# Jutho/KrylovKit.jl

Measured on NVIDIA H100. Metric: eigsolve_lanczos_operator_applications_per_sec, higher is better.
Workload: dtype f64

## Files before the change

krylovkit.jl_b200/csrc/basis.cu:

```cuda
#include "tsk.cuh"
#include <cmath>
#include <algorithm>

int32_t b2k_enqueue_dot(b2k_ctx* ctx, const void* q, void* x, int64_t n, const void* qprev,
                        int sprev_slot, int slot, int accum_slot);
int32_t b2k_enqueue_axpy_dev(b2k_ctx* ctx, void* x, const void* q, int s_slot, int64_t n);
int32_t b2k_enqueue_apply(b2k_ctx* ctx, const b2k_op* op, const VecRef& x, const VecRef& y,
                          double a0, double a1, bool shifted, const VecRef* dotv, int dot_slot);

using namespace tsk;

namespace {


template <typename T, bool UPDATE, bool PROJECT>
__global__ void __launch_bounds__(NTHREADS, 1)
k_phase(const __grid_constant__ PhaseParams<T> p, const __grid_constant__ ColList cl) {
    extern __shared__ __align__(128) uint8_t smem[];
    SmemView sm(smem);
    const int64_t ntiles = (p.n + Cfg<T>::R - 1) / Cfg<T>::R;
    const bool ragged = (p.n % Cfg<T>::R) != 0 && ((ntiles - 1) % gridDim.x) == blockIdx.x;
    pipe_setup(sm, ragged);
    Pipe st;
    if (threadIdx.x >= NCONS) producer_phase<T>(p, cl, sm, st);
    else consumer_phase<T, UPDATE, PROJECT>(p, sm, st);
}

template <typename T>
struct FusedParams {
    PhaseParams<T> ph[3];
    int32_t kind[3];
    int32_t nph;
    unsigned* barrier;
    unsigned barrier_base;
    const int* stop;
    FinalizeParams fin;
    PeerStep ps;
    unsigned long long* trace;
};

template <typename T>
__device__ __forceinline__ void peer_boundary(const FusedParams<T>& fp, int i, uint8_t* smem) {
    __threadfence();
    asm volatile("fence.proxy.async;" ::: "memory");
    __syncthreads();
    int* flag = reinterpret_cast<int*>(smem + OFF_RED + 256);
    if (threadIdx.x == 0) {
        const unsigned old = atomicAdd(fp.barrier, 1u);
        *flag = (old == fp.barrier_base + (unsigned)(i + 1) * gridDim.x - 1u);
    }
    __syncthreads();
    const PeerDev& pd = fp.ps.pd;
    const int tid = threadIdx.x;
    if (fp.ph[i].part_h == nullptr) {
        const unsigned long long sq = fp.ps.seq_norm;
        if (*flag && tid < 32) {
            __threadfence();
            double a = (tid < 16) ? partial_lane_sum(fp.ph[i].part_n, gridDim.x, 1, tid, 16) : 0.0;
            for (int o = 8; o > 0; o >>= 1) a += __shfl_xor_sync(0xffffffffu, a, o);
            if (tid == 0) peer_publish1(pd, PEER_CH_NORM, sq, a);
        }
        peer_wait(pd, PEER_CH_NORM, sq, tid);
        __syncthreads();
        return;
    }
    const unsigned long long seq = fp.ps.seq_coef[i];
    if (*flag && tid < NCONS) {
        __threadfence();
        const int k = fp.ph[i].k;
        const int L = coef_lanes(k);
        const int j = tid / L, l = tid % L;
        const bool valid = j < k;
        const double a = coef_colsum(fp.ph[i].part_h, gridDim.x, B2K_KSTRIDE, j, l, L, valid);
        if (valid && l == 0)
            for (int p = 0; p < pd.nranks; ++p) peer_slot(pd, p, PEER_CH_COEF, seq, pd.rank)[j] = a;
        __threadfence_system();
        named_bar_sync(1, NCONS);
        if (tid < pd.nranks) st_release_sys_u64(peer_flag(pd, tid, PEER_CH_COEF, seq, pd.rank), seq);
    }
    peer_wait(pd, PEER_CH_COEF, seq, tid);
    __syncthreads();
}

template <typename T>
__global__ void __launch_bounds__(NTHREADS, 1)
k_gs_fused(const __grid_constant__ FusedParams<T> fp, const __grid_constant__ ColList cl) {
    extern __shared__ __align__(128) uint8_t smem[];
    if (fp.stop && *reinterpret_cast<const volatile int*>(fp.stop)) {
        if (threadIdx.x == 0 && fp.nph > 1) atomicAdd(fp.barrier, (unsigned)(fp.nph - 1));
        return;
    }
    SmemView sm(smem);
    const bool tr0 = fp.trace && blockIdx.x == 0 && threadIdx.x == 0;
    if (tr0) b2k_trace(fp.trace, 10);
    const int64_t n = fp.ph[0].n;
    const int64_t ntiles = (n + Cfg<T>::R - 1) / Cfg<T>::R;
    const bool ragged = (n % Cfg<T>::R) != 0 && ((ntiles - 1) % gridDim.x) == blockIdx.x;
    pipe_setup(sm, ragged);
    Pipe st;
    const bool prod = threadIdx.x >= NCONS;
    if (fp.ps.on && fp.ps.seq_alpha && !prod) {
        peer_wait(fp.ps.pd, PEER_CH_ALPHA, fp.ps.seq_alpha, threadIdx.x);
        named_bar_sync(1, NCONS);
    }
    if (tr0) b2k_trace(fp.trace, 11);
    for (int i = 0; i < fp.nph; ++i) {
        if (prod) {
            producer_phase<T>(fp.ph[i], cl, sm, st);
        } else {
            if (fp.kind[i] == 0) consumer_phase<T, false, true>(fp.ph[i], sm, st);
            else if (fp.kind[i] == 1) consumer_phase<T, true, true>(fp.ph[i], sm, st);
            else consumer_phase<T, true, false>(fp.ph[i], sm, st);
        }
        if (tr0) b2k_trace(fp.trace, 12 + i);
        if (i + 1 < fp.nph) {
            if (fp.ps.on) peer_boundary<T>(fp, i, smem);
            else grid_barrier(fp.barrier, fp.barrier_base + (unsigned)(i + 1) * gridDim.x);
            if (tr0) b2k_trace(fp.trace, 15 + i);
        }
    }
    if (fp.fin.enabled && !prod) {
        double* sh = reinterpret_cast<double*>(smem + OFF_RED);
        int* flag = reinterpret_cast<int*>(smem + OFF_RED + 256);
        if (fp.ps.on) __threadfence_system();
        else __threadfence();
        named_bar_sync(1, NCONS);
        if (threadIdx.x == 0) {
            const unsigned t = atomicInc(fp.fin.ticket, gridDim.x - 1);
            *flag = (t == gridDim.x - 1);
        }
        named_bar_sync(1, NCONS);
        if (*flag) {
            __threadfence();
            if (fp.trace && threadIdx.x == 0) b2k_trace(fp.trace, 18);
            finalize_block(fp.fin, threadIdx.x, sh, fp.ps.on ? &fp.ps : nullptr);
            if (fp.trace && threadIdx.x == 0) b2k_trace(fp.trace, 19);
        }
    }
}

__global__ void __launch_bounds__(NCONS)
k_finalize(const double* __restrict__ A, const double* __restrict__ B, const double* __restrict__ N, int G,
           int stride, int k, double* __restrict__ res, int off, int noff) {
    __shared__ double sh[2];
    FinalizeParams f;
    f.A = A; f.B = B; f.N = N; f.G = G; f.stride = stride; f.k = k; f.res = res; f.off = off; f.noff = noff;
    f.rec = nullptr; f.alpha_col = -1; f.tol = 0.0; f.stop = nullptr; f.ticket = nullptr; f.enabled = 1;
    f.peer = 0; f.G_local = G; f.norm_done = 0;
    finalize_block(f, threadIdx.x, sh);
}

__global__ void k_lanczos_seed(double* rec, double beta, int* stop) {
    rec[2] = beta;
    rec[3] = 1.0 / beta;
    rec[4] = beta * beta;
    *stop = 0;
}

template <typename T>
__global__ void k_res_to_vec(const double* __restrict__ res, T* __restrict__ out, int k,
                             T alpha) {
    const int j = blockIdx.x * blockDim.x + threadIdx.x;
    if (j < k) out[j] = alpha * (T)res[j];
}

struct TransformParams {
    void* base;
    int64_t ld, n;
    int32_t m, keep, ldu;
    const double* U;
    int32_t u_in_smem;
};

constexpr int TR_OFF_U = NS * SLOT_BYTES;
constexpr int TR_U_BYTES = 232448 - TR_OFF_U - 256;
constexpr int TR_OFF_BAR = TR_OFF_U + TR_U_BYTES;
constexpr int TR_SMEM = TR_OFF_BAR + 2 * NS * 8;
constexpr int TJ = 36;
constexpr int TR_THREADS = NCONS + 32;

template <typename T, bool USM>
__global__ void __launch_bounds__(TR_THREADS, 1)
k_transform(const __grid_constant__ TransformParams p, const __grid_constant__ ColList cl) {
    using CF = Cfg<T>;
    using V16 = typename CF::V16;
    constexpr int R = CF::R, C = CF::C, VEC = CF::VEC;
    extern __shared__ __align__(128) uint8_t smem[];
    const uint32_t ring = smem_u32(smem);
    const uint32_t full = smem_u32(smem + TR_OFF_BAR), empty = full + NS * 8;
    T* Us = reinterpret_cast<T*>(smem + TR_OFF_U);
    const int pitch = ((p.keep + VEC - 1) / VEC) * VEC;
    if (threadIdx.x == 0) {
        for (int i = 0; i < NS; ++i) {
            mbar_init(full + 8 * i, 1);
            mbar_init(empty + 8 * i, NCONS / 32);
        }
        fence_mbar_init();
    }
// ... 779 lines not shown
    if (kind == 0) return launch_phase_t<T, false, true>(ctx, p, cl, grid);
    if (kind == 1) return launch_phase_t<T, true, true>(ctx, p, cl, grid);
    return launch_phase_t<T, true, false>(ctx, p, cl, grid);
}

template <typename T>
int grid_for_rows(const b2k_ctx* ctx, int64_t n) {
    int64_t ntiles = (n + Cfg<T>::R - 1) / Cfg<T>::R;
    if (ntiles < 1) ntiles = 1;
    return (int)std::min<int64_t>(ntiles, ctx->num_sms);
}

bool g_coop_launch = true;

template <typename T>
int32_t launch_fused(b2k_ctx* ctx, FusedParams<T>& fp, const ColList& cl, int grid) {
    fp.barrier = ctx->d_sync + 1;
    fp.barrier_base = ctx->barrier_base;
    ctx->barrier_base += (unsigned)(fp.nph - 1) * (unsigned)grid;
    void* args[] = {(void*)&fp, (void*)&cl};
    if (g_coop_launch)
        B2K_CUDA(ctx, cudaLaunchCooperativeKernel((const void*)k_gs_fused<T>, dim3(grid), dim3(NTHREADS),
                                                  args, SMEM_BYTES, ctx->stream));
    else
        k_gs_fused<T><<<grid, NTHREADS, SMEM_BYTES, ctx->stream>>>(fp, cl);
    B2K_LAUNCH_CHECK(ctx);
    return B2K_OK;
}

int32_t enqueue_finalize(b2k_ctx* ctx, const double* A, const double* B, const double* N, int G,
                         int k, int off, int noff) {
    if (k > NCONS) return b2k_fail(ctx, B2K_ENOTSUP, "finalize: more than %d coefficients per pass", NCONS);
    k_finalize<<<1, NCONS, 0, ctx->stream>>>(A, B, N, G, B2K_KSTRIDE, k, ctx->d_res, off, noff);
    B2K_LAUNCH_CHECK(ctx);
    return B2K_OK;
}

bool g_l2_hints = true;
int g_chain_mode = 0;

struct Panel {
    void* base;
    int64_t ld, n;
    int32_t sharded;
    std::vector<int32_t> idx;
};

int32_t make_panel(b2k_ctx* ctx, const b2k_vec* cols, int32_t k, Panel* pn) {
    int32_t sp = 0;
    B2K_TRY(b2k_resolve_cols(ctx, cols, k, &sp, &pn->idx));
    if (k == 0) {
        pn->base = nullptr;
        return B2K_OK;
    }
    const B2kSpace& s = ctx->spaces[sp];
    pn->base = s.base;
    pn->ld = s.ld;
    pn->n = s.n;
    pn->sharded = s.sharded;
    return B2K_OK;
}

template <typename T>
void fill_cols(ColList& cl, const std::vector<int32_t>& idx, int off, int cnt) {
    for (int i = 0; i < cnt; ++i) cl.c[i] = idx[off + i];
}

template <typename T>
PhaseParams<T> base_params(const Panel& pn, int k, const void* x, void* xout) {
    PhaseParams<T> p;
    memset(&p, 0, sizeof(p));
    p.base = (const T*)pn.base;
    p.ld = pn.ld;
    p.n = pn.n;
    p.k = k;
    p.x = (const T*)x;
    p.xout = (T*)xout;
    p.nvec = 1;
    p.beta_mode = 1;
    p.betax = (T)1;
    p.alphac = (T)1;
    p.l2_hints = g_l2_hints ? 1 : 0;
    return p;
}

template <typename T>
int32_t project_t(b2k_ctx* ctx, const Panel& pn, const VecRef& x, int k, int res_off) {
    const int grid = grid_for_rows<T>(ctx, pn.n);
    const int KC = kcap<T>();
    for (int off = 0; off < k; off += KC) {
        const int kk = std::min(KC, k - off);
        ColList cl;
        fill_cols<T>(cl, pn.idx, off, kk);
        PhaseParams<T> p = base_params<T>(pn, kk, x.ptr, nullptr);
        p.part_h = b2k_part_set(ctx, 0);
        const int pr = b2k_prof_begin(ctx, 3, (kk + 1.0) * sizeof(T) * (double)pn.n);
        B2K_TRY((launch_phase_t<T, false, true>(ctx, p, cl, grid)));
        b2k_prof_end(ctx, pr);
        B2K_TRY(enqueue_finalize(ctx, b2k_part_set(ctx, 0), nullptr, nullptr, grid, kk,
                                 res_off + off, 0));
    }
    return B2K_OK;
}

template <typename T>
int32_t unproject_t(b2k_ctx* ctx, const Panel& pn, const VecRef& y, int k, const double* dcoef,
                    const T* coef_t, double alpha, double beta, double* part_n) {
    const int grid = grid_for_rows<T>(ctx, pn.n);
    const int KC = kcap<T>();
    int off = 0;
    do {
        const int kk = std::min(KC, k - off);
        ColList cl;
        fill_cols<T>(cl, pn.idx, off, kk);
        PhaseParams<T> p = base_params<T>(pn, kk, y.ptr, y.ptr);
        p.store_x = 1;
        p.coef = dcoef ? dcoef + off : nullptr;
        p.coef_t = coef_t ? coef_t + off : nullptr;
        p.coef_sets = 1;
        p.coef_stride = 0;
        p.alphac = (T)alpha;
        if (off == 0) {
            p.beta_mode = beta == 0.0 ? 0 : (beta == 1.0 ? 1 : 2);
            p.betax = (T)beta;
        }
        p.part_n = (off + kk >= k) ? part_n : nullptr;
        const int pr = b2k_prof_begin(ctx, 4, (kk + 2.0) * sizeof(T) * (double)pn.n);
        B2K_TRY((launch_phase_t<T, true, false>(ctx, p, cl, grid)));
        b2k_prof_end(ctx, pr);
        off += kk;
    } while (off < k);
    return B2K_OK;
}

template <typename T>
int32_t cgs_fused_t(b2k_ctx* ctx, const Panel& pn, const VecRef& v, int k, int passes,
                    bool use_coop) {
    const int grid = grid_for_rows<T>(ctx, pn.n);
    ColList cl;
    fill_cols<T>(cl, pn.idx, 0, k);
    double* PA = b2k_part_set(ctx, 0);
    double* PB = b2k_part_set(ctx, 1);
    double* PN = b2k_part_set(ctx, 2);
    FusedParams<T> fp;
    memset(&fp, 0, sizeof(fp));
    int nph = 0;
    {
        PhaseParams<T> p = base_params<T>(pn, k, v.ptr, nullptr);
        p.part_h = PA;
        fp.ph[nph] = p; fp.kind[nph] = 0; ++nph;
    }
    if (passes == 2) {
        PhaseParams<T> p = base_params<T>(pn, k, v.ptr, v.ptr);
        p.store_x = 1;
        p.coef = PA; p.coef_sets = grid; p.coef_stride = B2K_KSTRIDE;
        p.alphac = (T)-1;
        p.part_h = PB;
        fp.ph[nph] = p; fp.kind[nph] = 1; ++nph;
    }
    {
        PhaseParams<T> p = base_params<T>(pn, k, v.ptr, v.ptr);
        p.store_x = 1;
        p.coef = (passes == 2) ? PB : PA; p.coef_sets = grid; p.coef_stride = B2K_KSTRIDE;
        p.alphac = (T)-1;
        p.part_n = PN;
        fp.ph[nph] = p; fp.kind[nph] = 2; ++nph;
// ... 292 lines not shown
    for (int j = 0; j < k; ++j) h_host[j] = ctx->h_res[j];
    nrm = sqrt(ctx->h_res[k]);
    if (nrm_out) *nrm_out = nrm;
    if (passes_out) *passes_out = passes;
    return B2K_OK;
}

extern "C" int32_t b2k_lanczos_expand(b2k_ctx* ctx, const b2k_op* op, const b2k_vec* cols,
                                      int32_t k, b2k_vec r, b2k_vec w, double beta_old,
                                      int32_t alg, double eta, double* alpha_out,
                                      double* beta_out) {
    if (!ctx || !op || !cols || k < 1 || !alpha_out || !beta_out) return B2K_EINVAL;
    if (alg < B2K_CGS || alg > B2K_MGS2B)
        return b2k_fail(ctx, B2K_EINVAL, "lanczos_expand: unknown orthogonalizer %d", alg);
    if (cols[k] != r) return b2k_fail(ctx, B2K_EINVAL, "lanczos_expand: cols[k] must be r");
    if (beta_old == 0.0) return b2k_fail(ctx, B2K_EINVAL, "lanczos_expand: beta_old == 0");
    Panel pn;
    B2K_TRY(make_panel(ctx, cols, k + 1, &pn));
    VecRef rv, rw, vprev;
    B2K_TRY(b2k_resolve(ctx, r, &rv));
    B2K_TRY(b2k_resolve(ctx, w, &rw));
    B2K_TRY(b2k_resolve(ctx, cols[k - 1], &vprev));
    if (rv.n != pn.n || rw.n != pn.n) return b2k_fail(ctx, B2K_EDIM, "lanczos_expand: length mismatch");
    for (int j = 0; j <= k; ++j)
        if (cols[j] == w) return b2k_fail(ctx, B2K_EINVAL, "lanczos_expand: w aliases the basis");
    const bool f64 = ctx->dtype == B2K_F64;
    const int K1 = k + 1;
    const double eps = f64 ? 2.220446049250313e-16 : 1.1920929e-07;
    const int S_H = 0;
    const int S_N = K1;
    const int S_A0 = K1 + 1;

    B2K_TRY(b2k_vec_scale(ctx, r, r, 1.0 / beta_old));

    if (alg == B2K_CGS || alg == B2K_CGS2 || alg == B2K_CGSIR) {
        B2K_TRY(b2k_enqueue_apply(ctx, op, rv, rw, 0.0, 1.0, false, &rv, S_A0));
        B2K_TRY(b2k_allreduce(ctx, ctx->d_res + S_A0, 1, pn.sharded));
        const bool one_pass = K1 <= (f64 ? kcap<double>() : kcap<float>());
        const bool defer_alpha = (alg == B2K_CGS2) && one_pass;
        double alpha = 0.0;
        if (!defer_alpha) {
            B2K_TRY(b2k_fetch_results(ctx, S_A0 + 1, 0));
            alpha = ctx->h_res[S_A0];
        }
        if (alg == B2K_CGS) {
            B2K_TRY(b2k_vec_axpy2(ctx, w, cols[k - 1], -beta_old, r, -alpha));
            B2K_TRY(b2k_enqueue_dot(ctx, nullptr, rw.ptr, pn.n, nullptr, -1, S_N, -1));
            B2K_TRY(b2k_allreduce(ctx, ctx->d_res + S_N, 1, pn.sharded));
            B2K_TRY(b2k_fetch_results(ctx, S_N + 1, 0));
            *alpha_out = alpha;
            *beta_out = sqrt(ctx->h_res[S_N]);
            return B2K_OK;
        }
        double ab2 = alpha * alpha + beta_old * beta_old;
        double beta = 0.0, nold = 0.0;
        bool first = true;
        for (;;) {
            const bool fusable = fused_ok(ctx, K1, pn.sharded, ctx->dtype);
            const bool prologue = first;
            if (alg == B2K_CGSIR && first) {
                B2K_TRY(b2k_vec_axpy2(ctx, w, cols[k - 1], -beta_old, r, -alpha));
                B2K_TRY(b2k_enqueue_dot(ctx, nullptr, rw.ptr, pn.n, nullptr, -1, S_N, -1));
                B2K_TRY(b2k_allreduce(ctx, ctx->d_res + S_N, 1, pn.sharded));
                B2K_TRY(b2k_fetch_results(ctx, S_N + 1, 0));
                beta = sqrt(ctx->h_res[S_N]);
                nold = sqrt(beta * beta + ab2);
                first = false;
                if (!(eps < beta && beta < eta * nold)) break;
                nold = beta;
                continue;
            }
            if (fusable) {
                const int grid = f64 ? grid_for_rows<double>(ctx, pn.n) : grid_for_rows<float>(ctx, pn.n);
                ColList cl;
                for (int i = 0; i < K1; ++i) cl.c[i] = pn.idx[i];
                double* PA = b2k_part_set(ctx, 0);
                double* PN = b2k_part_set(ctx, 2);
#define BUILD_AND_LAUNCH(T)                                                                   \
    {                                                                                         \
        FusedParams<T> fp;                                                                    \
        memset(&fp, 0, sizeof(fp));                                                           \
        PhaseParams<T> a = base_params<T>(pn, K1, rw.ptr, rw.ptr);                            \
        if (prologue) {                                                                       \
            a.nvec = 3; a.e1 = (const T*)vprev.ptr; a.e2 = (const T*)rv.ptr;                  \
            a.c1 = (T)(-beta_old); a.c2 = (T)(-alpha); a.store_x = 1;                         \
            if (defer_alpha) a.c2_dev = ctx->d_res + S_A0;                                    \
        }                                                                                     \
        a.part_h = PA;                                                                        \
        PhaseParams<T> c = base_params<T>(pn, K1, rw.ptr, rw.ptr);                            \
        c.store_x = 1; c.coef = PA; c.coef_sets = grid; c.coef_stride = B2K_KSTRIDE;          \
        c.alphac = (T)-1; c.part_n = PN;                                                      \
        fp.ph[0] = a; fp.kind[0] = 0; fp.ph[1] = c; fp.kind[1] = 2; fp.nph = 2;               \
        const int pr = b2k_prof_begin(ctx, 1, (2.0 * K1 + 3.0) * sizeof(T) * (double)pn.n);   \
        if (g_use_coop) { B2K_TRY(launch_fused<T>(ctx, fp, cl, grid)); }                      \
        else {                                                                                \
            B2K_TRY(launch_phase<T>(ctx, fp.ph[0], cl, 0, grid));                             \
            B2K_TRY(launch_phase<T>(ctx, fp.ph[1], cl, 2, grid));                             \
        }                                                                                     \
        b2k_prof_end(ctx, pr);                                                                \
    }
                if (f64) BUILD_AND_LAUNCH(double) else BUILD_AND_LAUNCH(float)
#undef BUILD_AND_LAUNCH
                B2K_TRY(enqueue_finalize(ctx, PA, nullptr, PN, grid, K1, S_H, S_N));
                B2K_TRY(b2k_fetch_results(ctx, S_A0 + 1, 0));
                if (defer_alpha) alpha = ctx->h_res[S_A0];
            } else if (one_pass) {
                const int grid = f64 ? grid_for_rows<double>(ctx, pn.n) : grid_for_rows<float>(ctx, pn.n);
                ColList cl;
                for (int i = 0; i < K1; ++i) cl.c[i] = pn.idx[i];
                double* PA = b2k_part_set(ctx, 0);
                double* PN = b2k_part_set(ctx, 2);
#define SPLIT_SWEEPS(T)                                                                       \
    {                                                                                         \
        PhaseParams<T> a = base_params<T>(pn, K1, rw.ptr, rw.ptr);                            \
        if (prologue) {                                                                       \
            a.nvec = 3; a.e1 = (const T*)vprev.ptr; a.e2 = (const T*)rv.ptr;                  \
            a.c1 = (T)(-beta_old); a.c2 = (T)(-alpha); a.store_x = 1;                         \
            if (defer_alpha) a.c2_dev = ctx->d_res + S_A0;                                    \
        }                                                                                     \
        a.part_h = PA;                                                                        \
        const int pr = b2k_prof_begin(ctx, 1, (2.0 * K1 + 3.0) * sizeof(T) * (double)pn.n);   \
        B2K_TRY(launch_phase<T>(ctx, a, cl, 0, grid));                                        \
        B2K_TRY(enqueue_finalize(ctx, PA, nullptr, nullptr, grid, K1, S_H, S_N));             \
        B2K_TRY(b2k_allreduce(ctx, ctx->d_res + S_H, K1, pn.sharded));                        \
        PhaseParams<T> c = base_params<T>(pn, K1, rw.ptr, rw.ptr);                            \
        c.store_x = 1; c.coef = ctx->d_res + S_H; c.coef_sets = 1; c.coef_stride = 0;         \
        c.alphac = (T)-1; c.part_n = PN;                                                      \
        B2K_TRY(launch_phase<T>(ctx, c, cl, 2, grid));                                        \
        b2k_prof_end(ctx, pr);                                                                \
    }
                if (f64) SPLIT_SWEEPS(double) else SPLIT_SWEEPS(float)
#undef SPLIT_SWEEPS
                k_finalize<<<1, NCONS, 0, ctx->stream>>>(PN, nullptr, PN, grid, B2K_KSTRIDE, 0, ctx->d_res, 0, S_N);
                B2K_LAUNCH_CHECK(ctx);
                B2K_TRY(b2k_allreduce(ctx, ctx->d_res + S_N, 1, pn.sharded));
                B2K_TRY(b2k_fetch_results(ctx, S_A0 + 1, 0));
                if (defer_alpha) alpha = ctx->h_res[S_A0];
            } else {
                if (prologue) B2K_TRY(b2k_vec_axpy2(ctx, w, cols[k - 1], -beta_old, r, -alpha));
                if (f64) B2K_TRY(cgs_pass_unfused_t<double>(ctx, pn, rw, K1, S_H, S_N));
                else B2K_TRY(cgs_pass_unfused_t<float>(ctx, pn, rw, K1, S_H, S_N));
                B2K_TRY(b2k_fetch_results(ctx, S_N + 1, 0));
            }
            alpha += ctx->h_res[S_H + k];
            beta = sqrt(ctx->h_res[S_N]);
            first = false;
            if (alg == B2K_CGS2) break;
            if (!(eps < beta && beta < eta * nold)) break;
            nold = beta;
        }
        *alpha_out = alpha;
        *beta_out = beta;
        return B2K_OK;
    }

    B2K_TRY(b2k_enqueue_apply(ctx, op, rv, rw, 0.0, 1.0, false, nullptr, -1));
    B2K_TRY(b2k_vec_axpby(ctx, w, cols[k - 1], -beta_old, 1.0));
    B2K_TRY(b2k_enqueue_dot(ctx, rv.ptr, rw.ptr, pn.n, nullptr, -1, S_A0, -1));
    B2K_TRY(b2k_allreduce(ctx, ctx->d_res + S_A0, 1, pn.sharded));
    B2K_TRY(b2k_enqueue_axpy_dev(ctx, rw.ptr, rv.ptr, S_A0, pn.n));
    double alpha = 0.0, beta = 0.0;
    if (alg == B2K_MGS) {
        B2K_TRY(b2k_enqueue_dot(ctx, nullptr, rw.ptr, pn.n, nullptr, -1, S_N, -1));
        B2K_TRY(b2k_allreduce(ctx, ctx->d_res + S_N, 1, pn.sharded));
        B2K_TRY(b2k_fetch_results(ctx, S_A0 + 1, 0));
        alpha = ctx->h_res[S_A0];
        beta = sqrt(ctx->h_res[S_N]);
    } else if (alg == B2K_MGS2B) {
        if (fused_ok(ctx, K1, pn.sharded, ctx->dtype)) {
            if (f64) B2K_TRY(cgs_fused_t<double>(ctx, pn, rw, K1, 1, g_use_coop));
            else B2K_TRY(cgs_fused_t<float>(ctx, pn, rw, K1, 1, g_use_coop));
        } else {
            if (f64) B2K_TRY(cgs_pass_unfused_t<double>(ctx, pn, rw, K1, S_H, S_N));
            else B2K_TRY(cgs_pass_unfused_t<float>(ctx, pn, rw, K1, S_H, S_N));
        }
        B2K_TRY(b2k_fetch_results(ctx, S_A0 + 1, 0));
        alpha = ctx->h_res[S_A0] + ctx->h_res[S_H + k];
        beta = sqrt(ctx->h_res[S_N]);
    } else if (alg == B2K_MGS2) {
        B2K_TRY(mgs_sweep(ctx, pn, rw, K1, S_H, -1));
        B2K_TRY(b2k_enqueue_dot(ctx, nullptr, rw.ptr, pn.n, nullptr, -1, S_N, -1));
        B2K_TRY(b2k_allreduce(ctx, ctx->d_res + S_N, 1, pn.sharded));
        B2K_TRY(b2k_fetch_results(ctx, S_A0 + 1, 0));
        alpha = ctx->h_res[S_A0] + ctx->h_res[S_H + k];
        beta = sqrt(ctx->h_res[S_N]);
    } else {
        B2K_TRY(b2k_enqueue_dot(ctx, nullptr, rw.ptr, pn.n, nullptr, -1, S_N, -1));
        B2K_TRY(b2k_allreduce(ctx, ctx->d_res + S_N, 1, pn.sharded));
        B2K_TRY(b2k_fetch_results(ctx, S_A0 + 1, 0));
        alpha = ctx->h_res[S_A0];
        beta = sqrt(ctx->h_res[S_N]);
        double nold = sqrt(beta * beta + alpha * alpha + beta_old * beta_old);
        while (eps < beta && beta < eta * nold) {
            nold = beta;
            B2K_TRY(mgs_sweep(ctx, pn, rw, K1, S_H, -1));
            B2K_TRY(b2k_enqueue_dot(ctx, nullptr, rw.ptr, pn.n, nullptr, -1, S_N, -1));
            B2K_TRY(b2k_allreduce(ctx, ctx->d_res + S_N, 1, pn.sharded));
            B2K_TRY(b2k_fetch_results(ctx, S_N + 1, 0));
            alpha += ctx->h_res[S_H + k];
            beta = sqrt(ctx->h_res[S_N]);
        }
    }
    *alpha_out = alpha;
    *beta_out = beta;
    return B2K_OK;
}

bool g_use_chain = true;

bool chain_ok(const b2k_ctx* ctx, const b2k_op* op, const b2k_vec* cols, int32_t k, int32_t nsteps, int32_t alg,
              double beta_old) {
    if (!g_use_chain || !g_use_coop || (alg != B2K_CGS2 && alg != B2K_MGS2B) || nsteps < 1 || nsteps > B2K_MAX_CHAIN)
        return false;
    int64_t op_rows = 0, op_cols = 0;
    int32_t op_kind = -1;
    if (b2k_op_info(op, &op_rows, &op_cols, nullptr, &op_kind) != B2K_OK) return false;
    if ((op_kind != 0 && op_kind != 2) || beta_old == 0.0 || !(beta_old == beta_old)) return false;
    const int32_t sp = B2K_VEC_SPACE(cols[k]);
    if (sp < 0 || sp >= (int32_t)ctx->spaces.size()) return false;
    const B2kSpace& s = ctx->spaces[sp];
    if (ctx->nranks > 1) {
        if (!s.sharded || !b2k_peer_ok(ctx) || !b2k_op_has_peer_halo(op) || op_rows != s.n) return false;
    } else if (op_rows != s.n || op_cols != s.n) {
        return false;
    }
    const int C = ctx->dtype == B2K_F64 ? 8 : 16;
    const int K1 = k + nsteps;
    return (K1 + C - 1) / C <= NS && K1 <= MAXCH * C && K1 <= PEER_SLOT;
}

template <typename T>
int32_t chain_step_gs(b2k_ctx* ctx, const Panel& pn, int K1, const VecRef& rw, const VecRef& vprev,
                      const VecRef& rv, double* rec_prev, double* rec, double tol, const PeerStep* psp,
                      bool scale_after) {
    const int grid = grid_for_rows<T>(ctx, pn.n);
    ColList cl;
    for (int i = 0; i < K1; ++i) cl.c[i] = pn.idx[i];
    double* PA = b2k_part_set(ctx, 0);
    double* PN = b2k_part_set(ctx, 2);
    FusedParams<T> fp;
    memset(&fp, 0, sizeof(fp));
    PhaseParams<T> a = base_params<T>(pn, K1, rw.ptr, rw.ptr);
    a.nvec = 3; a.e1 = (const T*)vprev.ptr; a.e2 = (const T*)rv.ptr; a.store_x = 1;
    a.c1_dev = rec_prev + 2;
    a.c2_dev = rec + 0;
    a.part_h = PA;
    PhaseParams<T> c = base_params<T>(pn, K1, rw.ptr, rw.ptr);
    c.store_x = 1; c.coef = PA; c.coef_sets = grid; c.coef_stride = B2K_KSTRIDE;
    c.alphac = (T)-1; c.part_n = PN;
    fp.ph[0] = a; fp.kind[0] = 0; fp.ph[1] = c; fp.kind[1] = 2; fp.nph = 2;
    if (scale_after) {
        PhaseParams<T> sc = base_params<T>(pn, 0, rw.ptr, rw.ptr);
        sc.store_x = 1; sc.beta_mode = 2; sc.scale_mode = 1;
        sc.scale_norm = PN; sc.scale_G = grid; sc.scale_stride = 1; sc.scale_tol = tol;
        fp.ph[2] = sc; fp.kind[2] = 2; fp.nph = 3;
    }
    fp.stop = reinterpret_cast<const int*>(ctx->d_sync + B2K_SYNC_STOP);
    fp.trace = ctx->d_trace;
    fp.fin.A = PA; fp.fin.B = nullptr; fp.fin.N = PN; fp.fin.G = grid; fp.fin.stride = B2K_KSTRIDE;
    fp.fin.k = K1; fp.fin.res = nullptr; fp.fin.off = 0; fp.fin.noff = 0; fp.fin.rec = rec;
    fp.fin.alpha_col = K1 - 1; fp.fin.tol = tol;
    fp.fin.stop = reinterpret_cast<int*>(ctx->d_sync + B2K_SYNC_STOP);
    fp.fin.ticket = ctx->d_sync + B2K_SYNC_GSFIN; fp.fin.enabled = 1;
    fp.fin.peer = 0; fp.fin.G_local = grid; fp.fin.norm_done = 0;
    if (psp && psp->on) {
        const PeerStep& ps = *psp;
        fp.ps = ps;
        char* win = b2k_peer_local(ctx);
        auto slot = [&](int ch, unsigned long long seq) {
            return reinterpret_cast<double*>(win + PEER_OFF_SLOTS) + (size_t)((ch * 2 + (int)(seq & 1ull)) * PEER_MAXR) * PEER_SLOT;
        };
        fp.ph[0].c2_dev = slot(PEER_CH_ALPHA, ps.seq_alpha);
        fp.ph[0].c2_sets = ps.pd.nranks;
        fp.ph[0].c2_stride = PEER_SLOT;
        fp.ph[1].coef = slot(PEER_CH_COEF, ps.seq_coef[0]);
        fp.ph[1].coef_sets = ps.pd.nranks;
        fp.ph[1].coef_stride = PEER_SLOT;
        fp.fin.A = fp.ph[1].coef; fp.fin.G = ps.pd.nranks; fp.fin.stride = PEER_SLOT; fp.fin.peer = 1;
        const int last = fp.nph - 1;
        if (scale_after) {
            fp.ph[2].scale_norm = slot(PEER_CH_NORM, ps.seq_norm);
            fp.ph[2].scale_G = ps.pd.nranks;
            fp.ph[2].scale_stride = PEER_SLOT;
            fp.fin.norm_done = 1;
        }
        if (ps.seq_halo) {
            fp.ph[last].send_lo = ps.send_lo;
            fp.ph[last].send_hi = ps.send_hi;
            fp.ph[last].halo_dn = ps.send_lo ? reinterpret_cast<T*>(ps.pd.win[ps.pd.rank - 1] + ps.dn_off) : nullptr;
            fp.ph[last].halo_up = ps.send_hi ? reinterpret_cast<T*>(ps.pd.win[ps.pd.rank + 1] + ps.up_off) : nullptr;
        }
    }
    const int pr = b2k_prof_begin(ctx, 1, (2.0 * K1 + 3.0) * sizeof(T) * (double)pn.n);
    B2K_TRY(launch_fused<T>(ctx, fp, cl, grid));
    b2k_prof_end(ctx, pr);
    return B2K_OK;
}

int32_t lanczos_chain(b2k_ctx* ctx, const b2k_op* op, b2k_vec* cols, int32_t k, int32_t nsteps,
                      double beta_old, double tol, int32_t alg, double* alphas_out, double* betas_out,
                      int32_t* steps_done, b2k_vec* r_out) {
    const bool f64 = ctx->dtype == B2K_F64;
    const int32_t space = B2K_VEC_SPACE(cols[k]);
    double* rec0 = ctx->d_steps;
    int* d_stop = reinterpret_cast<int*>(ctx->d_sync + B2K_SYNC_STOP);
    {
        VecRef t;
        for (int i = 0; i <= k; ++i) B2K_TRY(b2k_resolve(ctx, cols[i], &t));
    }
    k_lanczos_seed<<<1, 1, 0, ctx->stream>>>(rec0, beta_old, d_stop);
    B2K_LAUNCH_CHECK(ctx);
    const bool inplace = g_chain_mode == 1;
    std::vector<b2k_vec> touched, Vh, Wh;
    touched.push_back(cols[k]);
    int32_t enq = 0, rc = B2K_OK;
    const bool dist = ctx->nranks > 1;
    unsigned long long halo_seq = 0;
    if (inplace) B2K_TRY(b2k_vec_scale(ctx, cols[k], cols[k], 1.0 / beta_old));
    for (int32_t i = 0; i < nsteps; ++i) {
        const int32_t K = k + i;
        const b2k_vec R = cols[K];
        b2k_vec V = R, W = -1;
        if (!inplace) {
            rc = b2k_vec_alloc(ctx, space, &V);
            if (rc != B2K_OK) break;
            touched.push_back(V);
        }
        rc = b2k_vec_alloc(ctx, space, &W);
        if (rc != B2K_OK) break;
        touched.push_back(W);
        VecRef rR, rV, rW, vprev;
        rc = b2k_resolve(ctx, R, &rR);
        if (rc == B2K_OK) rc = b2k_resolve(ctx, V, &rV);
        if (rc == B2K_OK) rc = b2k_resolve(ctx, W, &rW);
        if (rc == B2K_OK) rc = b2k_resolve(ctx, cols[K - 1], &vprev);
        if (rc != B2K_OK) break;
        double* rec_prev = rec0 + (size_t)B2K_REC * i;
        double* rec = rec0 + (size_t)B2K_REC * (i + 1);
        const bool scale_after = inplace && (i + 1 < nsteps);
        SpmvFuse fz;
        memset(&fz, 0, sizeof(fz));
        if (!inplace) {
            fz.xscale = rec_prev + 3;
            fz.vout = rV.ptr;
        }
        fz.stop = d_stop;
        fz.dot_self = 1;
        fz.l2_hints = g_l2_hints ? 1 : 0;
        fz.trace = ctx->d_trace;
        if (alg == B2K_MGS2B) {
            fz.dot_sub_vec = vprev.ptr;
            fz.dot_sub_scale = rec_prev + 2;
        }
        PeerStep ps;
        memset(&ps, 0, sizeof(ps));
        if (dist) {
            ps.on = 1;
// ... 294 lines not shown
```

krylovkit.jl_b200/csrc/tsk.cuh:

```cuda
#pragma once
#include "common.cuh"

namespace tsk {

template <typename T> struct Cfg;
template <> struct Cfg<double> {
    static constexpr int R = 256, C = 8, VEC = 2;
    using V16 = double2;
    __device__ static __forceinline__ void unpack(const double2& v, double* o) { o[0] = v.x; o[1] = v.y; }
};
template <> struct Cfg<float> {
    static constexpr int R = 256, C = 16, VEC = 4;
    using V16 = float4;
    __device__ static __forceinline__ void unpack(const float4& v, float* o) {
        o[0] = v.x; o[1] = v.y; o[2] = v.z; o[3] = v.w;
    }
};

constexpr int NS = 12;
constexpr int NW = 3;
constexpr int NCONS = 256;
constexpr int NPROD = 4;
constexpr int NTHREADS = NCONS + 32 * NPROD;
constexpr int MAXCH = 16;
constexpr int SLOT_BYTES = 16384;
static_assert(NS % NPROD == 0, "a ring slot must always be refilled by the same producer warp");

template <typename T> constexpr int kcap() { return MAXCH * Cfg<T>::C; }

constexpr int OFF_RING = 0;
constexpr int OFF_WRING = NS * SLOT_BYTES;
constexpr int WSLOT_MAX = 3 * 256 * 8;
constexpr int OFF_W1 = OFF_WRING + NW * WSLOT_MAX;
constexpr int OFF_CS = OFF_W1 + 2 * 256 * 8;
constexpr int OFF_RED = OFF_CS + 1024;
constexpr int OFF_BAR = OFF_RED + 512;
constexpr int SMEM_BYTES = OFF_BAR + (2 * NS + 2 * NW) * 8;

struct ColList {
    int32_t c[256];
};

template <typename T>
struct PhaseParams {
    const T* base;
    int64_t ld;
    int64_t n;
    int32_t k;
    const T* x;
    T* xout;
    const T* e1;
    const T* e2;
    T c1, c2;
    const double* c1_dev;
    const double* c2_dev;
    int32_t c2_sets;
    int32_t c2_stride;
    T* halo_dn;
    T* halo_up;
    int64_t send_lo, send_hi;
    int32_t scale_mode;
    const double* scale_norm;
    int32_t scale_G, scale_stride;
    double scale_tol;
    int32_t nvec;
    int32_t store_x;
    int32_t l2_hints;
    const double* coef;
    const T* coef_t;
    int32_t coef_sets;
    int32_t coef_stride;
    T alphac, betax;
    int32_t beta_mode;
    double* part_h;
    double* part_n;
};

struct Pipe {
    uint32_t s = 0, ph = 0, ws = 0, wph = 0;
    uint32_t g = 0;
};

struct SmemView {
    uint8_t* raw;
    uint32_t ring, wring, full, empty, wfull, wempty;
    __device__ explicit SmemView(uint8_t* p) : raw(p) {
        ring = smem_u32(p + OFF_RING);
        wring = smem_u32(p + OFF_WRING);
        full = smem_u32(p + OFF_BAR);
        empty = full + NS * 8;
        wfull = empty + NS * 8;
        wempty = wfull + NW * 8;
    }
};

__device__ __forceinline__ void pipe_setup(const SmemView& sm, bool zero_ring) {
    if (threadIdx.x == 0) {
        for (int i = 0; i < NS; ++i) {
            mbar_init(sm.full + 8 * i, 1);
            mbar_init(sm.empty + 8 * i, NCONS / 32);
        }
        for (int i = 0; i < NW; ++i) {
            mbar_init(sm.wfull + 8 * i, 1);
            mbar_init(sm.wempty + 8 * i, NCONS / 32);
        }
        fence_mbar_init();
    }
    if (zero_ring) {
        uint4* q = reinterpret_cast<uint4*>(sm.raw);
        for (int i = threadIdx.x; i < OFF_CS / 16; i += blockDim.x) q[i] = make_uint4(0, 0, 0, 0);
        fence_proxy_async();
    }
    __syncthreads();
}

__device__ __forceinline__ int coef_lanes(int k) {
    int L = 16;
    while (L > 1 && L * k > NCONS) L >>= 1;
    return L;
}
__device__ __forceinline__ double partial_lane_sum(const double* P, int G, int stride, int l, int L) {
    double a = 0.0;
    int g = l;
    for (; g + 11 * L < G; g += 12 * L) {
        double t[12];
#pragma unroll
        for (int u = 0; u < 12; ++u) t[u] = __ldcg(P + (size_t)(g + u * L) * stride);
#pragma unroll
        for (int u = 0; u < 12; ++u) a += t[u];
    }
    for (; g + 3 * L < G; g += 4 * L) {
        const double t0 = __ldcg(P + (size_t)g * stride), t1 = __ldcg(P + (size_t)(g + L) * stride);
        const double t2 = __ldcg(P + (size_t)(g + 2 * L) * stride), t3 = __ldcg(P + (size_t)(g + 3 * L) * stride);
        a += t0; a += t1; a += t2; a += t3;
    }
    for (; g < G; g += L) a += __ldcg(P + (size_t)g * stride);
    return a;
}
__device__ __forceinline__ double coef_colsum(const double* P, int G, int stride, int j, int l, int L,
                                              bool valid) {
    double a = valid ? partial_lane_sum(P + j, G, stride, l, L) : 0.0;
    for (int o = L >> 1; o > 0; o >>= 1) a += __shfl_xor_sync(0xffffffffu, a, o);
    return a;
}

template <typename T>
__device__ __forceinline__ void producer_phase(const PhaseParams<T>& p, const ColList& cl,
                                               const SmemView& sm, Pipe& st) {
    using CF = Cfg<T>;
    constexpr int R = CF::R, C = CF::C;
    const int lane = threadIdx.x & 31;
    const uint32_t me = (threadIdx.x - NCONS) >> 5;
    const int nch = (p.k + C - 1) / C;
    const int64_t ntiles = (p.n + R - 1) / R;
    const uint64_t pol = p.l2_hints ? l2_policy_evict_first() : 0;
    for (int64_t tile = blockIdx.x; tile < ntiles; tile += gridDim.x) {
        const int64_t r0 = tile * R;
        const int rt = (int)((p.n - r0) < R ? (p.n - r0) : R);
        const uint32_t bytes = (uint32_t)((rt * sizeof(T) + 15) & ~(size_t)15);
        if (me == 0) {
            mbar_wait(sm.wempty + 8 * st.ws, st.wph ^ 1);
            if (lane == 0) mbar_expect_tx(sm.wfull + 8 * st.ws, bytes * (uint32_t)p.nvec);
            __syncwarp();
            if (lane < p.nvec) {
                const T* src = (lane == 0) ? p.x : (lane == 1 ? p.e1 : p.e2);
                bulk_g2s(sm.wring + st.ws * (3 * R * (int)sizeof(T)) + lane * R * (int)sizeof(T),
                         src + r0, bytes, sm.wfull + 8 * st.ws);
            }
        }
        if (++st.ws == NW) { st.ws = 0; st.wph ^= 1; }
        for (int c = 0; c < nch; ++c) {
            if ((st.g % NPROD) == me) {
                mbar_wait(sm.empty + 8 * st.s, st.ph ^ 1);
                const int ncol = (p.k - c * C) < C ? (p.k - c * C) : C;
                if (lane == 0) mbar_expect_tx(sm.full + 8 * st.s, bytes * (uint32_t)ncol);
                __syncwarp();
                if (lane < ncol) {
                    const T* src = p.base + (int64_t)cl.c[c * C + lane] * p.ld + r0;
                    if (p.l2_hints)
                        bulk_g2s_hint(sm.ring + st.s * SLOT_BYTES + lane * R * (int)sizeof(T), src, bytes,
                                      sm.full + 8 * st.s, pol);
                    else
                        bulk_g2s(sm.ring + st.s * SLOT_BYTES + lane * R * (int)sizeof(T), src, bytes,
                                 sm.full + 8 * st.s);
                }
            }
            ++st.g;
            if (++st.s == NS) { st.s = 0; st.ph ^= 1; }
        }
    }
}

template <typename T> struct VecOps;
template <> struct VecOps<double> {
    __device__ static __forceinline__ void fma_acc(double& acc, const double2& q, const double2& x) {
        acc = fma(q.x, x.x, acc);
        acc = fma(q.y, x.y, acc);
    }
};
template <> struct VecOps<float> {
    __device__ static __forceinline__ void fma_acc(float& acc, const float4& q, const float4& x) {
        acc = fmaf(q.x, x.x, acc);
        acc = fmaf(q.y, x.y, acc);
        acc = fmaf(q.z, x.z, acc);
        acc = fmaf(q.w, x.w, acc);
    }
};

template <typename T, bool UPDATE, bool PROJECT>
__device__ __forceinline__ void consumer_phase(const PhaseParams<T>& p, const SmemView& sm,
                                               Pipe& st) {
    using CF = Cfg<T>;
    using V16 = typename CF::V16;
    constexpr int R = CF::R, C = CF::C, VEC = CF::VEC;
    constexpr int CPW = C / 8;
    constexpr int NLD = R / (32 * VEC);
    const int tid = threadIdx.x;
    const int lane = tid & 31, w = tid >> 5;
    const int nch = (p.k + C - 1) / C;
    const int64_t ntiles = (p.n + R - 1) / R;
    T* cs = reinterpret_cast<T*>(sm.raw + OFF_CS);
    T* w1 = reinterpret_cast<T*>(sm.raw + OFF_W1);
    double* red = reinterpret_cast<double*>(sm.raw + OFF_RED);

    if (UPDATE) {
        if (p.coef_t) {
            for (int j = tid; j < p.k; j += NCONS) cs[j] = p.alphac * p.coef_t[j];
        } else {
            const int L = coef_lanes(p.k);
            const int j = tid / L, l = tid % L;
            const bool valid = j < p.k;
            const double h = coef_colsum(p.coef, p.coef_sets, p.coef_stride, j, l, L, valid);
            if (valid && l == 0) cs[j] = p.alphac * (T)h;
        }
        named_bar_sync(1, NCONS);
    }

    T acc_h[MAXCH][CPW];
#pragma unroll
    for (int c = 0; c < MAXCH; ++c)
#pragma unroll
        for (int cc = 0; cc < CPW; ++cc) acc_h[c][cc] = (T)0;
    T nrm = (T)0;
    int buf = 0;
    const uint64_t pol_last = p.l2_hints ? l2_policy_evict_last() : 0;
    T betax = p.betax;
    bool do_store = p.store_x != 0;
    if (UPDATE && p.scale_mode) {
        double* shn = reinterpret_cast<double*>(sm.raw + OFF_RED + 128);
        if (tid < 32) {
            double a;
            if (p.scale_stride == 1) {
                a = (tid < 16) ? partial_lane_sum(p.scale_norm, p.scale_G, 1, tid, 16) : 0.0;
                for (int o = 8; o > 0; o >>= 1) a += __shfl_xor_sync(0xffffffffu, a, o);
            } else {
                a = 0.0;
                for (int g = 0; g < p.scale_G; ++g)
                    a += *reinterpret_cast<const volatile double*>(p.scale_norm + (size_t)g * p.scale_stride);
            }
            if (tid == 0) shn[0] = a;
        }
        named_bar_sync(1, NCONS);
        const double beta = sqrt(shn[0]);
        if (beta <= p.scale_tol) do_store = false;
        betax = (T)(1.0 / beta);
    }
    T c1 = p.c1, c2 = p.c2;
    if (p.c1_dev) c1 = (T)(-(*reinterpret_cast<const volatile double*>(p.c1_dev)));
    if (p.c2_dev) {
        double a2 = 0.0;
        const int ns = p.c2_sets > 1 ? p.c2_sets : 1;
        for (int g = 0; g < ns; ++g)
            a2 += *reinterpret_cast<const volatile double*>(p.c2_dev + (size_t)g * p.c2_stride);
        c2 = (T)(-a2);
    }

    for (int64_t tile = blockIdx.x; tile < ntiles; tile += gridDim.x) {
        const int64_t r0 = tile * R;
        const int rt = (int)((p.n - r0) < R ? (p.n - r0) : R);
        mbar_wait(sm.wfull + 8 * st.ws, st.wph);
        const T* wv = reinterpret_cast<const T*>(sm.raw + OFF_WRING) + st.ws * 3 * R;
        T xv = wv[tid];
        if (p.nvec == 3) {
            xv = fma(c1, wv[R + tid], xv);
            xv = fma(c2, wv[2 * R + tid], xv);
        }
        if (tid >= rt) xv = (T)0;
        T acc = xv;
        const uint32_t s0 = st.s, ph0 = st.ph;
        if (UPDATE) {
            acc = (p.beta_mode == 0) ? (T)0 : (p.beta_mode == 1 ? xv : betax * xv);
            for (int c = 0; c < nch; ++c) {
                mbar_wait(sm.full + 8 * st.s, st.ph);
                const T* slot = reinterpret_cast<const T*>(sm.raw + OFF_RING + st.s * SLOT_BYTES);
                const int ncol = (p.k - c * C) < C ? (p.k - c * C) : C;
                if (ncol == C) {
                    T cv[C];
#pragma unroll
                    for (int i = 0; i < C / VEC; ++i)
                        CF::unpack(*reinterpret_cast<const V16*>(cs + c * C + i * VEC), cv + i * VEC);
#pragma unroll
                    for (int jj = 0; jj < C; ++jj) acc = fma(slot[jj * R + tid], cv[jj], acc);
                } else {
                    for (int jj = 0; jj < ncol; ++jj) acc = fma(slot[jj * R + tid], cs[c * C + jj], acc);
                }
                if (!PROJECT) {
                    __syncwarp();
                    if (lane == 0) mbar_arrive(sm.empty + 8 * st.s);
                }
                if (++st.s == NS) { st.s = 0; st.ph ^= 1; }
            }
            if (tid >= rt) acc = (T)0;
        }
        if (do_store && tid < rt) {
            if (p.l2_hints) st_hint(p.xout + r0 + tid, acc, pol_last);
            else p.xout[r0 + tid] = acc;
            if (UPDATE && !PROJECT) {
                const int64_t r = r0 + tid;
                if (p.halo_dn && r < p.send_lo) p.halo_dn[r] = acc;
                if (p.halo_up && r >= p.n - p.send_hi) p.halo_up[r - (p.n - p.send_hi)] = acc;
            }
        }
        if (p.part_n) nrm = fma(acc, acc, nrm);
        if (PROJECT) {
            T* wb = w1 + buf * R;
            wb[tid] = acc;
            named_bar_sync(1, NCONS);
            V16 xr[NLD];
#pragma unroll
            for (int i = 0; i < NLD; ++i)
                xr[i] = *reinterpret_cast<const V16*>(wb + VEC * lane + 32 * VEC * i);
            uint32_t ss = UPDATE ? s0 : st.s, pp = UPDATE ? ph0 : st.ph;
#pragma unroll
            for (int c = 0; c < MAXCH; ++c) {
                if (c < nch) {
                    if (!UPDATE) mbar_wait(sm.full + 8 * ss, pp);
                    const T* slot = reinterpret_cast<const T*>(sm.raw + OFF_RING + ss * SLOT_BYTES);
#pragma unroll
                    for (int cc = 0; cc < CPW; ++cc) {
                        const int cj = cc * 8 + w;
                        if (c * C + cj < p.k) {
                            const T* colp = slot + cj * R;
#pragma unroll
                            for (int i = 0; i < NLD; ++i) {
                                V16 q = *reinterpret_cast<const V16*>(colp + VEC * lane + 32 * VEC * i);
                                VecOps<T>::fma_acc(acc_h[c][cc], q, xr[i]);
                            }
                        }
                    }
                    __syncwarp();
                    if (lane == 0) mbar_arrive(sm.empty + 8 * ss);
                    if (++ss == NS) { ss = 0; pp ^= 1; }
                }
            }
            if (!UPDATE) { st.s = ss; st.ph = pp; }
            buf ^= 1;
        }
        __syncwarp();
        if (lane == 0) mbar_arrive(sm.wempty + 8 * st.ws);
        if (++st.ws == NW) { st.ws = 0; st.wph ^= 1; }
    }

    if (PROJECT) {
#pragma unroll
        for (int c = 0; c < MAXCH; ++c) {
#pragma unroll
            for (int cc = 0; cc < CPW; ++cc) {
                const int j = c * C + cc * 8 + w;
                double v = warp_sum((double)acc_h[c][cc]);
                if (c < nch && j < p.k && lane == 0)
                    p.part_h[(size_t)blockIdx.x * B2K_KSTRIDE + j] = v;
            }
        }
    }
    if (p.part_n) {
        double v = warp_sum((double)nrm);
        if (lane == 0) red[w] = v;
        named_bar_sync(1, NCONS);
        if (tid == 0) {
            double s = 0.0;
#pragma unroll
            for (int i = 0; i < NCONS / 32; ++i) s += red[i];
            p.part_n[blockIdx.x] = s;
        }
    }
}

struct FinalizeParams {
    const double* A;
    const double* B;
    const double* N;
    int G, stride, k;
    double* res;
    int off, noff;
    double* rec;
    int alpha_col;
    double tol;
    int* stop;
    unsigned* ticket;
    int enabled;
    int peer;
    int G_local;
    int norm_done;
};

__device__ __forceinline__ void finalize_block(const FinalizeParams& f, int tid, double* sh,
                                               const PeerStep* ps = nullptr) {
    double hval = 0.0;
    if (f.k > 0) {
        const int L = coef_lanes(f.k);
        const int j = tid / L, l = tid % L;
        const bool valid = j < f.k;
        double a = coef_colsum(f.A, f.G, f.stride, j, l, L, valid);
        if (f.B) a += coef_colsum(f.B, f.G, f.stride, j, l, L, valid);
        if (valid && l == 0) {
            if (f.res) f.res[f.off + j] = a;
            if (j == f.alpha_col) hval = a;
        }
        if (f.rec && valid && l == 0 && j == f.alpha_col) sh[0] = hval;
    }
    double n2 = 0.0;
    if (f.N && tid < 32) {
        double a = (tid < 16) ? partial_lane_sum(f.N, f.peer ? f.G_local : f.G, 1, tid, 16) : 0.0;
        for (int o = 8; o > 0; o >>= 1) a += __shfl_xor_sync(0xffffffffu, a, o);
        n2 = a;
    }
    double alpha0 = f.rec ? f.rec[0] : 0.0;
    if (f.peer && ps) {
        if (!f.norm_done) {
            if (tid == 0) peer_publish1(ps->pd, PEER_CH_NORM, ps->seq_norm, n2);
            peer_wait(ps->pd, PEER_CH_NORM, ps->seq_norm, tid);
        }
        named_bar_sync(1, NCONS);
        if (tid == 0) {
            n2 = peer_sum1(ps->pd, PEER_CH_NORM, ps->seq_norm, 0);
            if (ps->seq_alpha) alpha0 = peer_sum1(ps->pd, PEER_CH_ALPHA, ps->seq_alpha, 0);
            if (ps->seq_halo) {
                __threadfence_system();
                if (ps->send_lo) st_relaxed_sys_u64(peer_hflag(ps->pd, ps->pd.rank - 1, ps->seq_halo, 1), ps->seq_halo);
                if (ps->send_hi) st_relaxed_sys_u64(peer_hflag(ps->pd, ps->pd.rank + 1, ps->seq_halo, 0), ps->seq_halo);
            }
        }
    }
    if (f.N && tid == 0 && f.res) f.res[f.noff] = n2;
    if (f.rec) {
        named_bar_sync(1, NCONS);
        if (tid == 0) {
            f.rec[0] = alpha0;
            const double alpha = alpha0 + sh[0];
            const double beta = sqrt(n2);
            f.rec[1] = alpha;
            f.rec[2] = beta;
            f.rec[3] = 1.0 / beta;
            f.rec[4] = n2;
            if (f.stop && beta <= f.tol) *f.stop = 1;
        }
    }
}

__device__ __forceinline__ void grid_barrier(unsigned* counter, unsigned target) {
    __threadfence();
    asm volatile("fence.proxy.async;" ::: "memory");
    __syncthreads();
    if (threadIdx.x == 0) {
        atomicAdd(counter, 1u);
        while ((int)(*(volatile unsigned*)counter - target) < 0) {
        }
        __threadfence();
    }
    __syncthreads();
}

}
```

Baseline: 337.6.

## Reuse prologue vectors from shared memory and decouple producers from grid barrier

In the fused Gram-Schmidt kernel, the last two basis columns (the previous and current Lanczos vectors already staged in the prologue working buffer) are now read from shared memory instead of being re-fetched by bulk copy in both the projection and update phases. The phase-boundary grid barrier now synchronizes only the consumer warps via a named barrier, and producers wait on a new shared-memory mbarrier (xready) before starting the next phase. This is meant to cut global memory traffic for two columns per phase and let producers avoid full-block syncs. It adds synchronization complexity, with a risk of ordering bugs between the stored x and the producer prefetch.

```diff
diff --git a/krylovkit.jl_b200/csrc/basis.cu b/krylovkit.jl_b200/csrc/basis.cu
--- a/krylovkit.jl_b200/csrc/basis.cu
+++ b/krylovkit.jl_b200/csrc/basis.cu
@@ -41,15 +41,12 @@
 
 template <typename T>
 __device__ __forceinline__ void peer_boundary(const FusedParams<T>& fp, int i, uint8_t* smem) {
-    __threadfence();
-    asm volatile("fence.proxy.async;" ::: "memory");
-    __syncthreads();
     int* flag = reinterpret_cast<int*>(smem + OFF_RED + 256);
     if (threadIdx.x == 0) {
         const unsigned old = atomicAdd(fp.barrier, 1u);
         *flag = (old == fp.barrier_base + (unsigned)(i + 1) * gridDim.x - 1u);
     }
-    __syncthreads();
+    named_bar_sync(1, NCONS);
     const PeerDev& pd = fp.ps.pd;
     const int tid = threadIdx.x;
     if (fp.ph[i].part_h == nullptr) {
@@ -61,11 +58,11 @@
             if (tid == 0) peer_publish1(pd, PEER_CH_NORM, sq, a);
         }
         peer_wait(pd, PEER_CH_NORM, sq, tid);
-        __syncthreads();
+        named_bar_sync(1, NCONS);
         return;
     }
     const unsigned long long seq = fp.ps.seq_coef[i];
-    if (*flag && tid < NCONS) {
+    if (*flag) {
         __threadfence();
         const int k = fp.ph[i].k;
         const int L = coef_lanes(k);
@@ -79,7 +76,7 @@
         if (tid < pd.nranks) st_release_sys_u64(peer_flag(pd, tid, PEER_CH_COEF, seq, pd.rank), seq);
     }
     peer_wait(pd, PEER_CH_COEF, seq, tid);
-    __syncthreads();
+    named_bar_sync(1, NCONS);
 }
 
 template <typename T>
@@ -104,16 +101,25 @@
         named_bar_sync(1, NCONS);
     }
     if (tr0) b2k_trace(fp.trace, 11);
+    bool stored = false;
+    uint32_t xph = 0;
     for (int i = 0; i < fp.nph; ++i) {
         if (prod) {
+            if (stored) {
+                if (threadIdx.x < NCONS + 32) mbar_wait(sm.xready, xph);
+                xph ^= 1u;
+            }
             producer_phase<T>(fp.ph[i], cl, sm, st);
-        } else {
-            if (fp.kind[i] == 0) consumer_phase<T, false, true>(fp.ph[i], sm, st);
-            else if (fp.kind[i] == 1) consumer_phase<T, true, true>(fp.ph[i], sm, st);
-            else consumer_phase<T, true, false>(fp.ph[i], sm, st);
-        }
+            stored = stored || fp.ph[i].store_x;
+            continue;
+        }
+        if (fp.kind[i] == 0) consumer_phase<T, false, true>(fp.ph[i], sm, st);
+        else if (fp.kind[i] == 1) consumer_phase<T, true, true>(fp.ph[i], sm, st);
+        else consumer_phase<T, true, false>(fp.ph[i], sm, st);
+        stored = stored || fp.ph[i].store_x;
         if (tr0) b2k_trace(fp.trace, 12 + i);
         if (i + 1 < fp.nph) {
+            boundary_enter(sm, stored);
             if (fp.ps.on) peer_boundary<T>(fp, i, smem);
             else grid_barrier(fp.barrier, fp.barrier_base + (unsigned)(i + 1) * gridDim.x);
             if (tr0) b2k_trace(fp.trace, 15 + i);
@@ -1059,6 +1065,20 @@
     p.alphac = (T)1;
     p.l2_hints = g_l2_hints ? 1 : 0;
     return p;
+}
+
+template <typename T>
+void set_prologue(PhaseParams<T>& p, const VecRef& vprev, const VecRef& v) {
+    p.nvec = 3;
+    p.pro_tail = 1;
+    p.e1 = (const T*)vprev.ptr;
+    p.e2 = (const T*)v.ptr;
+}
+template <typename T>
+void copy_prologue(PhaseParams<T>& dst, const PhaseParams<T>& src) {
+    dst.nvec = src.nvec; dst.pro_tail = src.pro_tail; dst.e1 = src.e1; dst.e2 = src.e2;
+    dst.c1 = src.c1; dst.c2 = src.c2; dst.c1_dev = src.c1_dev; dst.c2_dev = src.c2_dev;
+    dst.c2_sets = src.c2_sets; dst.c2_stride = src.c2_stride;
 }
 
 template <typename T>
@@ -1517,12 +1537,13 @@
         memset(&fp, 0, sizeof(fp));                                                           \
         PhaseParams<T> a = base_params<T>(pn, K1, rw.ptr, rw.ptr);                            \
         if (prologue) {                                                                       \
-            a.nvec = 3; a.e1 = (const T*)vprev.ptr; a.e2 = (const T*)rv.ptr;                  \
-            a.c1 = (T)(-beta_old); a.c2 = (T)(-alpha); a.store_x = 1;                         \
+            set_prologue<T>(a, vprev, rv);                                                    \
+            a.c1 = (T)(-beta_old); a.c2 = (T)(-alpha);                                        \
             if (defer_alpha) a.c2_dev = ctx->d_res + S_A0;                                    \
         }                                                                                     \
         a.part_h = PA;                                                                        \
         PhaseParams<T> c = base_params<T>(pn, K1, rw.ptr, rw.ptr);                            \
+        copy_prologue<T>(c, a);                                                               \
         c.store_x = 1; c.coef = PA; c.coef_sets = grid; c.coef_stride = B2K_KSTRIDE;          \
         c.alphac = (T)-1; c.part_n = PN;                                                      \
         fp.ph[0] = a; fp.kind[0] = 0; fp.ph[1] = c; fp.kind[1] = 2; fp.nph = 2;               \
@@ -1549,8 +1570,8 @@
     {                                                                                         \
         PhaseParams<T> a = base_params<T>(pn, K1, rw.ptr, rw.ptr);                            \
         if (prologue) {                                                                       \
-            a.nvec = 3; a.e1 = (const T*)vprev.ptr; a.e2 = (const T*)rv.ptr;                  \
-            a.c1 = (T)(-beta_old); a.c2 = (T)(-alpha); a.store_x = 1;                         \
+            set_prologue<T>(a, vprev, rv);                                                    \
+            a.c1 = (T)(-beta_old); a.c2 = (T)(-alpha);                                        \
             if (defer_alpha) a.c2_dev = ctx->d_res + S_A0;                                    \
         }                                                                                     \
         a.part_h = PA;                                                                        \
@@ -1559,6 +1580,7 @@
         B2K_TRY(enqueue_finalize(ctx, PA, nullptr, nullptr, grid, K1, S_H, S_N));             \
         B2K_TRY(b2k_allreduce(ctx, ctx->d_res + S_H, K1, pn.sharded));                        \
         PhaseParams<T> c = base_params<T>(pn, K1, rw.ptr, rw.ptr);                            \
+        copy_prologue<T>(c, a);                                                               \
         c.store_x = 1; c.coef = ctx->d_res + S_H; c.coef_sets = 1; c.coef_stride = 0;         \
         c.alphac = (T)-1; c.part_n = PN;                                                      \
         B2K_TRY(launch_phase<T>(ctx, c, cl, 2, grid));                                        \
@@ -1676,11 +1698,12 @@
     FusedParams<T> fp;
     memset(&fp, 0, sizeof(fp));
     PhaseParams<T> a = base_params<T>(pn, K1, rw.ptr, rw.ptr);
-    a.nvec = 3; a.e1 = (const T*)vprev.ptr; a.e2 = (const T*)rv.ptr; a.store_x = 1;
+    set_prologue<T>(a, vprev, rv);
     a.c1_dev = rec_prev + 2;
     a.c2_dev = rec + 0;
     a.part_h = PA;
     PhaseParams<T> c = base_params<T>(pn, K1, rw.ptr, rw.ptr);
+    copy_prologue<T>(c, a);
     c.store_x = 1; c.coef = PA; c.coef_sets = grid; c.coef_stride = B2K_KSTRIDE;
     c.alphac = (T)-1; c.part_n = PN;
     fp.ph[0] = a; fp.kind[0] = 0; fp.ph[1] = c; fp.kind[1] = 2; fp.nph = 2;
@@ -1705,9 +1728,11 @@
         auto slot = [&](int ch, unsigned long long seq) {
             return reinterpret_cast<double*>(win + PEER_OFF_SLOTS) + (size_t)((ch * 2 + (int)(seq & 1ull)) * PEER_MAXR) * PEER_SLOT;
         };
-        fp.ph[0].c2_dev = slot(PEER_CH_ALPHA, ps.seq_alpha);
-        fp.ph[0].c2_sets = ps.pd.nranks;
-        fp.ph[0].c2_stride = PEER_SLOT;
+        for (int i = 0; i < 2; ++i) {
+            fp.ph[i].c2_dev = slot(PEER_CH_ALPHA, ps.seq_alpha);
+            fp.ph[i].c2_sets = ps.pd.nranks;
+            fp.ph[i].c2_stride = PEER_SLOT;
+        }
         fp.ph[1].coef = slot(PEER_CH_COEF, ps.seq_coef[0]);
         fp.ph[1].coef_sets = ps.pd.nranks;
         fp.ph[1].coef_stride = PEER_SLOT;
diff --git a/krylovkit.jl_b200/csrc/tsk.cuh b/krylovkit.jl_b200/csrc/tsk.cuh
--- a/krylovkit.jl_b200/csrc/tsk.cuh
+++ b/krylovkit.jl_b200/csrc/tsk.cuh
@@ -35,7 +35,7 @@
 constexpr int OFF_CS = OFF_W1 + 2 * 256 * 8;
 constexpr int OFF_RED = OFF_CS + 1024;
 constexpr int OFF_BAR = OFF_RED + 512;
-constexpr int SMEM_BYTES = OFF_BAR + (2 * NS + 2 * NW) * 8;
+constexpr int SMEM_BYTES = OFF_BAR + (2 * NS + 2 * NW + 1) * 8;
 
 struct ColList {
     int32_t c[256];
@@ -64,6 +64,7 @@
     int32_t scale_G, scale_stride;
     double scale_tol;
     int32_t nvec;
+    int32_t pro_tail;
     int32_t store_x;
     int32_t l2_hints;
     const double* coef;
@@ -83,7 +84,7 @@
 
 struct SmemView {
     uint8_t* raw;
-    uint32_t ring, wring, full, empty, wfull, wempty;
+    uint32_t ring, wring, full, empty, wfull, wempty, xready;
     __device__ explicit SmemView(uint8_t* p) : raw(p) {
         ring = smem_u32(p + OFF_RING);
         wring = smem_u32(p + OFF_WRING);
@@ -91,6 +92,7 @@
         empty = full + NS * 8;
         wfull = empty + NS * 8;
         wempty = wfull + NW * 8;
+        xready = wempty + NW * 8;
     }
 };
 
@@ -104,6 +106,7 @@
             mbar_init(sm.wfull + 8 * i, 1);
             mbar_init(sm.wempty + 8 * i, NCONS / 32);
         }
+        mbar_init(sm.xready, 1);
         fence_mbar_init();
     }
     if (zero_ring) {
@@ -173,9 +176,10 @@
             if ((st.g % NPROD) == me) {
                 mbar_wait(sm.empty + 8 * st.s, st.ph ^ 1);
                 const int ncol = (p.k - c * C) < C ? (p.k - c * C) : C;
-                if (lane == 0) mbar_expect_tx(sm.full + 8 * st.s, bytes * (uint32_t)ncol);
+                const int nld = p.pro_tail ? max(0, min(ncol, p.k - 2 - c * C)) : ncol;
+                if (lane == 0) mbar_expect_tx(sm.full + 8 * st.s, bytes * (uint32_t)nld);
                 __syncwarp();
-                if (lane < ncol) {
+                if (lane < nld) {
                     const T* src = p.base + (int64_t)cl.c[c * C + lane] * p.ld + r0;
                     if (p.l2_hints)
                         bulk_g2s_hint(sm.ring + st.s * SLOT_BYTES + lane * R * (int)sizeof(T), src, bytes,
@@ -294,7 +298,8 @@
                 mbar_wait(sm.full + 8 * st.s, st.ph);
                 const T* slot = reinterpret_cast<const T*>(sm.raw + OFF_RING + st.s * SLOT_BYTES);
                 const int ncol = (p.k - c * C) < C ? (p.k - c * C) : C;
-                if (ncol == C) {
+                const int tail0 = p.pro_tail ? p.k - 2 - c * C : C;
+                if (ncol == C && tail0 >= C) {
                     T cv[C];
 #pragma unroll
                     for (int i = 0; i < C / VEC; ++i)
@@ -302,7 +307,10 @@
 #pragma unroll
                     for (int jj = 0; jj < C; ++jj) acc = fma(slot[jj * R + tid], cv[jj], acc);
                 } else {
-                    for (int jj = 0; jj < ncol; ++jj) acc = fma(slot[jj * R + tid], cs[c * C + jj], acc);
+                    for (int jj = 0; jj < ncol; ++jj) {
+                        const T q = jj < tail0 ? slot[jj * R + tid] : wv[(jj - tail0 + 1) * R + tid];
+                        acc = fma(q, cs[c * C + jj], acc);
+                    }
                 }
                 if (!PROJECT) {
                     __syncwarp();
@@ -339,8 +347,10 @@
 #pragma unroll
                     for (int cc = 0; cc < CPW; ++cc) {
                         const int cj = cc * 8 + w;
-                        if (c * C + cj < p.k) {
+                        const int j = c * C + cj;
+                        if (j < p.k) {
                             const T* colp = slot + cj * R;
+                            if (p.pro_tail && j >= p.k - 2) colp = wv + (j - p.k + 3) * R;
 #pragma unroll
                             for (int i = 0; i < NLD; ++i) {
                                 V16 q = *reinterpret_cast<const V16*>(colp + VEC * lane + 32 * VEC * i);
@@ -458,17 +468,21 @@
     }
 }
 
-__device__ __forceinline__ void grid_barrier(unsigned* counter, unsigned target) {
+__device__ __forceinline__ void boundary_enter(const SmemView& sm, bool signal) {
     __threadfence();
     asm volatile("fence.proxy.async;" ::: "memory");
-    __syncthreads();
+    named_bar_sync(1, NCONS);
+    if (signal && threadIdx.x == 0) mbar_arrive(sm.xready);
+}
+
+__device__ __forceinline__ void grid_barrier(unsigned* counter, unsigned target) {
     if (threadIdx.x == 0) {
         atomicAdd(counter, 1u);
         while ((int)(*(volatile unsigned*)counter - target) < 0) {
         }
         __threadfence();
     }
-    __syncthreads();
-}
-
-}
+    named_bar_sync(1, NCONS);
+}
+
+}
```

After: 346.7, median of 6. +2.7%, better.
